# cczls1991/DL_Biomass

Hardware: NVIDIA B200
Metric: train tree-clouds/sec @10k pts (higher is better)
Workload: dtype bf16

## Files before the change

### dl_biomass_b200/csrc/sa_tc.cu

```cuda
#include <cuda.h>
#include <math.h>

#include "tc_common.cuh"

namespace b2pn {
namespace tc {

constexpr int R = 128;
constexpr int KC = 64;
constexpr int NUM_EPI = 256;
constexpr int NUM_LOAD = 128;
constexpr int LOAD_GROUPS = 2;
constexpr int MMA_WARP = (NUM_EPI + LOAD_GROUPS * NUM_LOAD) / 32;
constexpr int NT = NUM_EPI + LOAD_GROUPS * NUM_LOAD + 32;
constexpr int NT_TMA = 2 * NUM_EPI + 64;
constexpr int PROD_WARP_TMA = MMA_WARP + 1;
constexpr int NT_WIDE = 2 * NUM_EPI + 32 + NUM_LOAD;
constexpr int B_BYTES = R * LINE_BYTES;

constexpr unsigned GI_NONE = 0x00ffffffu;
__device__ __forceinline__ int gi_seg(unsigned b) { return (int)(b & 0xffffffu); }
__device__ __forceinline__ bool gi_none(unsigned b) { return (b & 0xffffffu) == 0xffffffu; }
__device__ __forceinline__ int gi_slot0(unsigned b) { return (int)((b >> 24) & 7u) << 3; }
__device__ __forceinline__ int gi_nv(unsigned b) { return (int)((b >> 27) & 15u); }
// ... 422 lines not shown
#pragma unroll
        for (int b = 0; b < 2; ++b) {
            const int64_t r8 = r0 + b * 64;
            qraw2[b] = __ldg(src.rm.rgrp + (r8 >> 3));
            qdead2 |= (r8 >= src.rm.rows ? 1u : 0u) << b;
        }
    }
    __device__ __forceinline__ void no_tile() { qraw2[0] = qraw2[1] = GI_NONE, qdead2 = 3u; }
    __device__ __forceinline__ void shift_tiles()
    {
#pragma unroll
        for (int b = 0; b < 2; ++b) qraw1[b] = qraw2[b];
        qdead1 = qdead2;
    }
    __device__ __forceinline__ void advance_tile()
    {
#pragma unroll
        for (int b = 0; b < 2; ++b) qinf[b] = (((qdead1 >> b) & 1u) || gi_none(qraw1[b])) ? GI_NONE : qraw1[b];
    }
    __device__ __forceinline__ void prefetch_next_rows(int lt, int kc0, int kstep, int num_kc) const
    {
        if ((lt & 7) != 0) return;
#pragma unroll
        for (int b = 0; b < 2; ++b) {
            const unsigned w = qraw1[b];
            if (((qdead1 >> b) & 1u) || gi_none(w) || gi_nv(w) == 0 || gi_slot0(w) != 0) continue;
            const int64_t base = (int64_t)gi_seg(w) * src.C + (lt & 15) * 4;
            for (int kc = kc0; kc < num_kc; kc += kstep) {
                if (kc * KC + (lt & 15) * 4 >= src.C) break;
                asm volatile("prefetch.global.L2 [%0];" ::"l"(src.arg + base + kc * KC));
                asm volatile("prefetch.global.L2 [%0];" ::"l"(src.dout + base + kc * KC));
            }
        }
    }
    __device__ __forceinline__ void load(int kc, int lt, Item &it) const
    {
        const int ch4 = kc * KC + (lt & 15) * 4;
        it.first = 0u;
#pragma unroll
        for (int b = 0; b < 2; ++b) {
            src.load_quad(qinf[b], ch4, it.q[b]);
            it.first |= (src.starts(qinf[b], ch4) ? 1u : 0u) << b;
        }
    }
    __device__ __forceinline__ void store(uint8_t *B, int kc, int lt, const Item &it) const
    {
        const int ch4 = kc * KC + (lt & 15) * 4;
#pragma unroll
        for (int b = 0; b < 2; ++b)
            src.store_quad(it.q[b], (it.first >> b) & 1u, ch4, lt >> 4, smem_u32(B) + b * (64 * LINE_BYTES), (lt & 15) * 4);
    }
    __device__ __forceinline__ void begin_tile(int64_t tile, int lt)
    {
        row0 = tile * R + (lt & 1) * 64;
        if (src.rm.seg_mode) {
#pragma unroll
            for (int g = 0; g < 8; ++g) inf[g] = src.rm.info(row0 + g * 8);
        } else {
#pragma unroll
            for (int g = 0; g < 8; ++g) inf[g] = src.rm.info_slots(row0 + g * 8);
        }
    }
    __device__ __forceinline__ void produce(uint8_t *B, int kc, int lt) const
    {
        const int cl = lt >> 1, nb = lt & 1;
        uint8_t *dst = B + nb * (64 * LINE_BYTES);
        const int ch = kc * KC + cl;
        uint4 v[8];
#pragma unroll
        for (int g = 0; g < 8; ++g) v[g] = src.chunk_i(ch, row0 + g * 8, inf[g]);
#pragma unroll
        for (int g = 0; g < 8; ++g) *reinterpret_cast<uint4 *>(dst + line_chunk_off(cl, g)) = v[g];
    }
    static __device__ __forceinline__ uint64_t b_desc(uint32_t b_saddr, int ks)
    {
        return smem_desc_sw128(b_saddr + ks * (16 * LINE_BYTES), 64 * LINE_BYTES, ATOM_BYTES);
    }
};

struct TmaFeatLoader {
    static constexpr bool B_MN = true;
    static constexpr bool USES_TMA = true;
    static constexpr bool WIDE = true;
    __device__ __forceinline__ void resolve(int64_t) {}
    __device__ __forceinline__ void begin_tile(int64_t, int) {}
    __device__ __forceinline__ void produce_tma(uint8_t *B, int64_t tile, int kc, const TmaMap *map, uint64_t *bar) const
    {
        mbar_expect_tx(bar, B_BYTES);
        tma_load_2d(B, map, (int)(tile * R), kc * KC, bar);
        tma_load_2d(B + 64 * LINE_BYTES, map, (int)(tile * R + 64), kc * KC, bar);
    }
    static __device__ __forceinline__ uint64_t b_desc(uint32_t b_saddr, int ks)
    {
        return smem_desc_sw128(b_saddr + ks * (16 * LINE_BYTES), 64 * LINE_BYTES, ATOM_BYTES);
    }
};

struct EpCtx {
    uint8_t *stage;
    const TmaMap *m0;
    const TmaMap *m1;
    uint64_t *bar;
    int64_t next_tile;
    int next_ch;
};
constexpr int EPI_STAGE_PER_WARP = 2 * 32 * LINE_BYTES;

__device__ __forceinline__ void stage_chunk(uint8_t *tile32, int lane, int g, const uint4 &v)
{
    *reinterpret_cast<uint4 *>(tile32 + lane * LINE_BYTES + ((g ^ (lane & 7)) << 4)) = v;
}
__device__ __forceinline__ uint4 unstage_chunk(const uint8_t *tile32, int lane, int g)
{
    return *reinterpret_cast<const uint4 *>(tile32 + lane * LINE_BYTES + ((g ^ (lane & 7)) << 4));
}

struct StoreF32Ep {
    static constexpr bool STAGED = false;
    float *out;
    int C;
    int64_t ld;
    __device__ __forceinline__ void resolve(int64_t) {}
    __device__ __forceinline__ void begin() {}
    __device__ __forceinline__ void tile_mt(uint32_t taddr, int64_t tile, int ch, int mt, int half, const EpCtx &cx)
    {
#pragma unroll 1
        for (int cc = half * 2; cc < half * 2 + 2; ++cc) {
            float v[32];
            tmem_ld32(taddr + cc * 32, v);
            if (ch < C) {
                float4 *dst = reinterpret_cast<float4 *>(out + (int64_t)ch * ld + tile * R + cc * 32);
#pragma unroll
                for (int j = 0; j < 8; ++j) dst[j] = make_float4(v[4 * j], v[4 * j + 1], v[4 * j + 2], v[4 * j + 3]);
            }
        }
    }
    __device__ __forceinline__ void finish_mt(int ch, int mt, int half) {}
};

template <int MT>
struct StatsEpTC {
    static constexpr bool STAGED = false;
    int C;
    double *partial;
    int cpad;
    int nslot;
    double S[MT], Q[MT];
    __device__ __forceinline__ void resolve(int64_t) {}
    __device__ __forceinline__ void begin()
    {
#pragma unroll
        for (int i = 0; i < MT; ++i) S[i] = Q[i] = 0.0;
    }
    __device__ __forceinline__ void tile_mt(uint32_t taddr, int64_t tile, int ch, int mt, int half, const EpCtx &cx)
    {
        float s = 0.f, q = 0.f;
#pragma unroll 1
        for (int cc = half * 2; cc < half * 2 + 2; ++cc) {
            float v[32];
            tmem_ld32(taddr + cc * 32, v);
#pragma unroll
            for (int j = 0; j < 32; ++j) {
                s += v[j];
                q = fmaf(v[j], v[j], q);
            }
        }
        S[mt] += (double)s;
        Q[mt] += (double)q;
    }
    __device__ __forceinline__ void finish_mt(int ch, int mt, int slot)
    {
        if (ch < C) {
            double *pt = partial + ((int64_t)blockIdx.x * nslot + slot) * 2 * cpad;
            pt[ch] = S[mt];
            pt[cpad + ch] = Q[mt];
        }
    }
};

// ... 269 lines not shown
        float *st = reinterpret_cast<float *>(cx.stage);
        __syncwarp();
#pragma unroll 1
        for (int cc = 0; cc < 2; ++cc) {
            float v[32];
            tmem_ld32(taddr + (half * 2 + cc) * 32, v);
#pragma unroll
            for (int j = 0; j < 32; ++j) {
                const int r = cc * 32 + j;
                st[r * 32 + ((((lane >> 2) ^ (r & 7))) << 2) + (lane & 3)] = v[j];
            }
        }
        __syncwarp();
        const bool vec = (C & 3) == 0;
#pragma unroll 1
        for (int rr = 0; rr < 2; ++rr) {
            const int r = rr * 32 + lane;
            const int64_t row = tile * R + half * 64 + r;
            if (row >= rm.rows) continue;
            int64_t dst = row;
            if (!rm.seg_mode) {
                const int sidx = __ldg(rm.row_src + row);
                if (sidx < 0) continue;
                dst = sidx;
            }
            float *base = dx + dst * C + ch0;
#pragma unroll
            for (int c4 = 0; c4 < 8; ++c4) {
                if (ch0 + c4 * 4 >= C) break;
                const float4 q = *reinterpret_cast<const float4 *>(st + r * 32 + ((c4 ^ (r & 7)) << 2));
                if (dxi != nullptr && !rm.seg_mode) {
                    const float e[4] = {q.x, q.y, q.z, q.w};
                    unsigned long long *acc = reinterpret_cast<unsigned long long *>(dxi + dst * C + ch0 + c4 * 4);
#pragma unroll
                    for (int k = 0; k < 4; ++k) {
                        if (ch0 + c4 * 4 + k >= C) break;
                        if (e[k] != 0.f) atomicAdd(acc + k, (unsigned long long)__float2ll_rn(e[k] * FIXED_ONE));
                    }
                } else if (vec) {
                    if (rm.seg_mode) {
                        *reinterpret_cast<float4 *>(base + c4 * 4) = q;
                    } else if (q.x != 0.f || q.y != 0.f || q.z != 0.f || q.w != 0.f) {
                        asm volatile("red.global.add.v4.f32 [%0], {%1, %2, %3, %4};" ::"l"(base + c4 * 4), "f"(q.x), "f"(q.y), "f"(q.z),
                                     "f"(q.w)
                                     : "memory");
                    }
                } else {
                    const float e[4] = {q.x, q.y, q.z, q.w};
#pragma unroll
                    for (int k = 0; k < 4; ++k) {
                        if (ch0 + c4 * 4 + k >= C) break;
                        if (rm.seg_mode) base[c4 * 4 + k] = e[k];
                        else if (e[k] != 0.f) atomicAdd(base + c4 * 4 + k, e[k]);
                    }
                }
            }
        }
    }
    __device__ __forceinline__ void finish_mt(int ch, int mt, int half) {}
};

template <int MT, bool STAGED, bool TMA>
struct SmemPlan {
    static constexpr int A_BYTES = MT * 128 * LINE_BYTES;
    static constexpr int STAGE_BYTES = A_BYTES + B_BYTES;
    static constexpr int EPI_WARPS = (TMA ? 2 : 1) * (NUM_EPI / 32);
    static constexpr int STAGES = !STAGED ? (MT == 1 ? 5 : 4) : (TMA ? (MT == 1 ? 3 : 2) : (MT == 1 ? 4 : 3));
    static constexpr int EPI_OFF = STAGES * STAGE_BYTES;
    static constexpr int EPI_BYTES = STAGED ? EPI_WARPS * EPI_STAGE_PER_WARP : 0;
    static constexpr int BAR_OFF = EPI_OFF + EPI_BYTES;
    static constexpr int TOTAL = BAR_OFF + 256 + 1024;
};

template <class BL, class = void>
struct LoaderPipelined { static constexpr bool value = false; };
template <class BL>
struct LoaderPipelined<BL, decltype((void)BL::PIPELINED)> { static constexpr bool value = BL::PIPELINED; };

template <class BL, class = void>
struct LoaderGroupsWide { static constexpr int value = 1; };
template <class BL>
struct LoaderGroupsWide<BL, decltype((void)BL::PIPE_GROUPS)> { static constexpr int value = BL::PIPELINED ? BL::PIPE_GROUPS : 1; };
template <class BL>
constexpr int gemm_threads() { return BL::USES_TMA ? NT_TMA : (BL::WIDE ? NT_WIDE + (LoaderGroupsWide<BL>::value - 1) * NUM_LOAD : NT); }

template <int MT, class BL, class EP>
__global__ void __launch_bounds__(gemm_threads<BL>(), 1)
    tc_rows_gemm_kernel(const GemmParams gp, BL bl, EP ep, const __grid_constant__ TmaMap tmap, const __grid_constant__ TmaMap tmap_e0,
                        const __grid_constant__ TmaMap tmap_e1)
{
    constexpr bool TMA = BL::USES_TMA;
    constexpr bool WIDE = BL::WIDE;
    static_assert(!TMA || WIDE, "TMA-fed kernels use the wide layout");
    constexpr int EPI_GROUPS = WIDE ? 2 : 1;
    constexpr int EPI_WARPS = EPI_GROUPS * (NUM_EPI / 32);
    constexpr int LGROUPS = WIDE ? LoaderGroupsWide<BL>::value : LOAD_GROUPS;
    constexpr int LOAD_T0 = WIDE ? (MMA_WARP + 1) * 32 : NUM_EPI;
    constexpr int NLOAD = NUM_LOAD;
    using P = SmemPlan<MT, EP::STAGED, WIDE>;
    extern __shared__ uint8_t smem_raw[];
    uint8_t *smem = reinterpret_cast<uint8_t *>((reinterpret_cast<uintptr_t>(smem_raw) + 1023) & ~(uintptr_t)1023);
    uint64_t *full = reinterpret_cast<uint64_t *>(smem + P::BAR_OFF);
    uint64_t *empty = full + P::STAGES;
    uint64_t *tfull = empty + P::STAGES;
    uint64_t *tempty = tfull + 2;
    uint64_t *ebar = tempty + 2;
    uint32_t *tmem_holder = reinterpret_cast<uint32_t *>(ebar + EPI_WARPS);

    const int tid = threadIdx.x, warp = tid >> 5, lane = tid & 31;
    const int mg = blockIdx.y;
    constexpr int TCOLS = MT * R * 2;
    const int64_t rows = gp.rows_dev ? *gp.rows_dev : gp.rows;
    const int64_t num_tiles = (rows + R - 1) / R;
    bl.resolve(rows);
    ep.resolve(rows);

    if (tid == 0) {
        for (int s = 0; s < P::STAGES; ++s) {
            mbar_init(&full[s], TMA ? 1 : NLOAD);
            mbar_init(&empty[s], 1);
        }
        for (int a = 0; a < 2; ++a) {
            mbar_init(&tfull[a], 1);
            mbar_init(&tempty[a], NUM_EPI);
        }
        for (int w = 0; w < EPI_WARPS; ++w) mbar_init(&ebar[w], 1);
        fence_barrier_init();
    }
    if (warp == MMA_WARP) tmem_alloc<TCOLS>(tmem_holder);
    tc_fence_before();
    __syncthreads();
    tc_fence_after();
    const uint32_t tmem_base = *tmem_holder;

    if (TMA && warp == PROD_WARP_TMA) {
        if constexpr (TMA) {
            if (lane == 0) {
                uint32_t it = 0;
                for (int64_t tile = blockIdx.x; tile < num_tiles; tile += gridDim.x) {
                    for (int kc = 0; kc < gp.num_kc; ++kc, ++it) {
                        const int s = it % P::STAGES;
                        const uint32_t ph = (it / P::STAGES) & 1u;
                        mbar_wait(&empty[s], ph ^ 1u);
                        uint8_t *A = smem + s * P::STAGE_BYTES;
                        uint8_t *B = A + P::A_BYTES;
                        mbar_expect_tx(&full[s], P::A_BYTES);
                        bulk_g2s(A, gp.a_packed + ((int64_t)mg * gp.num_kc + kc) * P::A_BYTES, P::A_BYTES, &full[s]);
                        bl.produce_tma(B, tile, kc, &tmap, &full[s]);
                        mbar_arrive(&full[s]);
                    }
                }
            }
        }
    } else if (!TMA && tid >= LOAD_T0 && tid < LOAD_T0 + LGROUPS * NLOAD) {
        if constexpr (!TMA) {
            const int g = (tid - LOAD_T0) / NLOAD;
            const int lt = (tid - LOAD_T0) % NLOAD;
            if constexpr (LoaderPipelined<BL>::value) {
                typename BL::Item cur, nxt;
                const int num_kc = gp.num_kc;
                const int64_t my_tiles = blockIdx.x < num_tiles ? (num_tiles - blockIdx.x + gridDim.x - 1) / gridDim.x : 0;
                const int64_t items = my_tiles * num_kc;
                const int tstep = num_kc >= LGROUPS ? 1 : LGROUPS / num_kc;
                auto tile_of = [&](int64_t tl) { return (int64_t)blockIdx.x + tl * gridDim.x; };
                auto fetch_or_none = [&](int64_t tl) {
                    if (tl < my_tiles) bl.fetch_tile(tile_of(tl), lt);
                    else bl.no_tile();
                };
                int64_t i = g;
                if (i < items) {
                    int64_t tl = i / num_kc;
                    int kc = (int)(i % num_kc);
                    bl.fetch_tile(tile_of(tl), lt);
                    bl.shift_tiles();
                    bl.advance_tile();
                    bl.load(kc, lt, cur);
                    fetch_or_none(tl + tstep);
                    bl.shift_tiles();
                    bl.prefetch_next_rows(lt, num_kc % LGROUPS == 0 ? g : 0, num_kc % LGROUPS == 0 ? LGROUPS : 1, num_kc);
                    fetch_or_none(tl + 2 * tstep);
                    auto item = [&](typename BL::Item &c, typename BL::Item &n) -> bool {
                        const int64_t ni = i + LGROUPS;
                        const bool has_next = ni < items;
                        int nkc = kc + LGROUPS;
                        int64_t ntl = tl;
                        while (nkc >= num_kc) {
                            nkc -= num_kc;
                            ++ntl;
                        }
                        if (has_next) {
                            if (ntl != tl) bl.advance_tile();
                            bl.load(nkc, lt, n);
                            if (ntl != tl) {
                                bl.shift_tiles();
                                bl.prefetch_next_rows(lt, num_kc % LGROUPS == 0 ? g : 0, num_kc % LGROUPS == 0 ? LGROUPS : 1, num_kc);
                                fetch_or_none(ntl + 2 * tstep);
                            }
                        }
                        const int s = (int)(i % P::STAGES);
                        const uint32_t ph = (uint32_t)(i / P::STAGES) & 1u;
                        mbar_wait(&empty[s], ph ^ 1u);
                        uint8_t *A = smem + s * P::STAGE_BYTES;
                        uint8_t *B = A + P::A_BYTES;
                        if (lt == 0) {
                            mbar_expect_tx(&full[s], P::A_BYTES);
                            bulk_g2s(A, gp.a_packed + ((int64_t)mg * num_kc + kc) * P::A_BYTES, P::A_BYTES, &full[s]);
                        }
                        RouteSource::zero_tile<NLOAD>(smem_u32(B), B_BYTES, lt);
                        RouteSource::group_barrier<NLOAD>(1 + g);
                        bl.store(B, kc, lt, c);
                        fence_proxy_async_smem();
                        mbar_arrive(&full[s]);
                        i = ni;
                        kc = nkc;
                        tl = ntl;
                        return has_next;
                    };
                    while (item(cur, nxt) && item(nxt, cur)) {
                    }
                }
            } else {
                uint32_t it = 0;
                int64_t cur_tile = -1;
                for (int64_t tile = blockIdx.x; tile < num_tiles; tile += gridDim.x) {
                    for (int kc = 0; kc < gp.num_kc; ++kc, ++it) {
                        if ((int)(it % LGROUPS) != g) continue;
                        if (tile != cur_tile) {
                            bl.begin_tile(tile, lt);
                            cur_tile = tile;
                        }
                        const int s = it % P::STAGES;
                        const uint32_t ph = (it / P::STAGES) & 1u;
                        mbar_wait(&empty[s], ph ^ 1u);
// ... 685 lines not shown
        bn[c] = (float)mean;
        bn[cmax + c] = (float)rstd;
        bn[2 * cmax + c] = (float)scale;
        bn[3 * cmax + c] = (float)((double)beta[c] - mean * scale);
    }
}

__global__ void bn_bwd_finalize_tc_kernel(const double *partial, int gx, int C, int cpad, const CountArg count, int training,
                                          float *grad_gamma, float *grad_beta, float *sbar)
{
    const int c = (blockIdx.x * blockDim.x + threadIdx.x) >> 5;
    if (c >= C) return;
    double S, Q;
    warp_sum_partials(partial, gx, cpad, c, S, Q);
    if ((threadIdx.x & 31) == 0) {
        const double E = count.get();
        if (grad_beta) grad_beta[c] = (float)S;
        if (grad_gamma) grad_gamma[c] = (float)Q;
        sbar[c] = (training && E > 0) ? (float)(S / E) : 0.f;
        sbar[C + c] = (training && E > 0) ? (float)(Q / E) : 0.f;
    }
}

template <bool CLOUDS>
__global__ void route_grad_tc_kernel(RowMapTC rm, const int64_t *rows_dev, const float *dout, const int32_t *arg, int C, int64_t ld,
                                     __nv_bfloat16 *dh)
{
    if (rows_dev) rm.rows = *rows_dev;
    const int64_t groups = (rm.rows + 127) / 128 * 16;
    const int64_t total = groups * C;
    for (int64_t i = (int64_t)blockIdx.x * blockDim.x + threadIdx.x; i < total; i += (int64_t)gridDim.x * blockDim.x) {
        const int ch = (int)(i / groups);
        const int64_t g = i - (int64_t)ch * groups;
        const unsigned inf = rm.info(g * 8);
        uint4 v = make_uint4(0u, 0u, 0u, 0u);
        if (CLOUDS) {
            float f[8];
            bool any = false;
#pragma unroll
            for (int e = 0; e < 8; ++e) {
                const int64_t row = g * 8 + e;
                f[e] = 0.f;
                if (e < gi_nv(inf)) {
                    const int64_t sg = __ldg(rm.batch + row);
                    if ((int64_t)__ldg(arg + sg * C + ch) == row) {
                        f[e] = __ldg(dout + sg * C + ch);
                        any = true;
                    }
                }
            }
            if (any) v = pack8(f);
        } else if (gi_nv(inf) > 0) {
            const int64_t m = gi_seg(inf);
            const int a = __ldg(arg + m * C + ch) - gi_slot0(inf);
            if (a >= 0 && a < 8) {
                const unsigned short gb = __bfloat16_as_ushort(__float2bfloat16(__ldg(dout + m * C + ch)));
                const unsigned w = (a & 1) ? ((unsigned)gb << 16) : (unsigned)gb;
                const int q = a >> 1;
                v.x = q == 0 ? w : 0u;
                v.y = q == 1 ? w : 0u;
                v.z = q == 2 ? w : 0u;
                v.w = q == 3 ? w : 0u;
            }
        }
        *reinterpret_cast<uint4 *>(dh + (int64_t)ch * ld + g * 8) = v;
    }
}

__global__ void bn_bwd_apply_tc_kernel(RowMapTC rm, const int64_t *rows_dev, __nv_bfloat16 *dz, const __nv_bfloat16 *z, int C,
                                       int64_t ld, const float *scale, const float *sbar)
{
    if (rows_dev) rm.rows = *rows_dev;
    const int64_t groups = (rm.rows + 127) / 128 * 16;
    const int64_t total = groups * C;
    for (int64_t i = (int64_t)blockIdx.x * blockDim.x + threadIdx.x; i < total; i += (int64_t)gridDim.x * blockDim.x) {
        const int ch = (int)(i / groups);
        const int64_t r8 = (i - (int64_t)ch * groups) * 8;
        const int nv = rm.valid8(r8);
        uint4 *p = reinterpret_cast<uint4 *>(dz + (int64_t)ch * ld + r8);
        if (nv == 0) {
            *p = make_uint4(0u, 0u, 0u, 0u);
            continue;
        }
        float d[8], zf[8];
        unpack8(*p, d);
        unpack8h(__ldg(reinterpret_cast<const uint4 *>(z + (int64_t)ch * ld + r8)), zf);
        const float sc = scale[ch];
        const float s1 = sbar[ch], s2 = sbar[C + ch];
#pragma unroll
        for (int e = 0; e < 8; ++e) d[e] = e < nv ? sc * (d[e] - s1 - zf[e] * s2) : 0.f;
        *p = pack8(d);
    }
}

struct DwReduceJob {
    const float *partial;
    int splits, n_out, k_total, use_map;
    InCols cols;
    int k_true, ones_idx;
    float *grad_w, *grad_b;
};
struct DwReduceJobs {
    DwReduceJob j[3];
};
__global__ void dw_reduce_flat_tc_kernel(const DwReduceJobs jobs)
{
    const DwReduceJob &jb = jobs.j[blockIdx.y];
    const int k_true = jb.k_true, k_total = jb.k_total, n_out = jb.n_out, splits = jb.splits;
    const int64_t i = (int64_t)blockIdx.x * blockDim.x + threadIdx.x;
    if (i >= (int64_t)n_out * (k_true + 1)) return;
    const int n = (int)(i / (k_true + 1));
    const int k = (int)(i - (int64_t)n * (k_true + 1));
    int c0 = -1, c1 = -1;
    if (k == k_true) {
        c0 = jb.ones_idx;
    } else if (!jb.use_map) {
        c0 = k;
    } else {
        const int nx = jb.cols.nx();
        if (k < jb.cols.c_in) {
            c0 = k;
            c1 = jb.cols.x_f32 ? k + jb.cols.c_in : -1;
        } else {
            c0 = nx + (k - jb.cols.c_in);
            c1 = c0 + 3;
        }
    }
    const int64_t stride = (int64_t)n_out * k_total;
    const float *base = jb.partial + (int64_t)n * k_total;
    constexpr int U = 16;
    double acc[U];
#pragma unroll
    for (int u = 0; u < U; ++u) acc[u] = 0.0;
    int p = 0;
    for (; p + U <= splits; p += U) {
#pragma unroll
        for (int u = 0; u < U; ++u) {
            const float *row = base + (int64_t)(p + u) * stride;
            float v = row[c0];
            if (c1 >= 0) v += row[c1];
            acc[u] += (double)v;
        }
    }
    for (; p < splits; ++p) {
        const float *row = base + (int64_t)p * stride;
        acc[0] += (double)row[c0];
        if (c1 >= 0) acc[0] += (double)row[c1];
    }
#pragma unroll
    for (int w = U / 2; w > 0; w >>= 1)
#pragma unroll
        for (int u = 0; u < w; ++u) acc[u] += acc[u + w];
    const double sum = acc[0];
    if (k == k_true) {
        if (jb.grad_b) jb.grad_b[n] = (float)sum;
    } else if (jb.grad_w) {
        jb.grad_w[(int64_t)n * k_true + k] = (float)sum;
    }
}

constexpr int DWR_WARPS = 8;
constexpr int DWR_MAX_SPLITS = 160;
__global__ void __launch_bounds__(32 * DWR_WARPS) dw_reduce_tc_kernel(const DwReduceJobs jobs)
{
    const DwReduceJob &jb = jobs.j[blockIdx.y];
    const int k_true = jb.k_true, k_total = jb.k_total, n_out = jb.n_out, splits = jb.splits;
    const int w = threadIdx.y;
    const int64_t i = (int64_t)blockIdx.x * 32 + threadIdx.x;
    const bool live = i < (int64_t)n_out * (k_true + 1);
    const int n = live ? (int)(i / (k_true + 1)) : 0;
    const int k = live ? (int)(i - (int64_t)n * (k_true + 1)) : 0;
    int c0 = 0, c1 = -1;
    if (k == k_true) {
        c0 = jb.ones_idx;
// ... 562 lines not shown
    for (int i = 0; i < 3; ++i) {
        dj.j[i] = jobs[i < n ? i : 0];
        const int64_t tot = (int64_t)dj.j[i].n_out * (dj.j[i].k_true + 1);
        mx = tot > mx ? tot : mx;
    }
    if (mx <= 16384)
        dw_reduce_tc_kernel<<<dim3((unsigned)((mx + 31) / 32), (unsigned)n), dim3(32, DWR_WARPS), 0, st>>>(dj);
    else
        dw_reduce_flat_tc_kernel<<<dim3((unsigned)((mx + 127) / 128), (unsigned)n), 128, 0, st>>>(dj);
    note_launch();
}

int sa_backward_bf16(const b2pn_sa_args &a, const b2pn_sa_grads &g, cudaStream_t st)
{
    int rc = check_args_tc(a);
    if (rc) return rc;
    if (!g.grad_out) return B2PN_EINVAL;
    const ShapesTC s = shapes_tc(a);
    if (a.n_dst == 0 || s.rows == 0) return B2PN_OK;
    if (a.workspace_bytes < sa_workspace_bytes_bf16(a, 1) || !a.workspace) return B2PN_EINVAL;
    WsTC ws(a.workspace);
    BwdWsTC b = carve_bwd_tc(a, s, ws);
    const RowMapTC rm = rowmap_tc(a, s);
    const RowsArg ra = rowsarg_tc(a, s);
    const __nv_bfloat16 *z1 = (const __nv_bfloat16 *)a.h1, *z2 = (const __nv_bfloat16 *)a.h2;
    float *bn1 = a.bn, *bn2 = a.bn + 4 * s.cmax;
    const bool need_dx = g.grad_x != nullptr && a.c_in > 0;

    {
        const PackJob jobs[3] = {pack_job(a.mlp.w[2], s.c2, s.c3, 1, s.c2, nullptr, b.pkT[2]),
                                 pack_job(a.mlp.w[1], s.c1, s.c2, 1, s.c1, nullptr, b.pkT[1]),
                                 pack_job(a.mlp.w[0], a.c_in, s.c1, 1, s.c0, nullptr, b.pkT[0])};
        launch_packs(jobs, need_dx ? 3 : 2, st);
    }
    const CountArg count = {a.seg_mode == B2PN_SEG_SLOTS ? a.num_rows + 1 : nullptr, (double)s.rows};

    MaskSumsStoreEpTC<1> e31 = {s.c2, a.mlp.gamma[1], a.mlp.beta[1], a.mlp.act, b.partial, s.cpad, 4};
    MaskSumsStoreEpTC<2> e32 = {s.c2, a.mlp.gamma[1], a.mlp.beta[1], a.mlp.act, b.partial, s.cpad, 4};
    TmaMap mdz2, mz2;
    if ((rc = make_tma_feature_major(&mdz2, b.dz2, s.c2, s.ld, 32))) return rc;
    if ((rc = make_tma_feature_major(&mz2, z2, s.c2, s.ld, 32))) return rc;
    LineFillK<FeatSource<1>> xa2 = {{rm, z2, s.c2, s.ld, a.mlp.act, s.c2, a.mlp.gamma[1], a.mlp.beta[1], FMT_BF16}};
    TmaMap map_v = kNoMap, map_a1 = kNoMap, map_a2 = kNoMap;
    const bool tma_x = a.row_valid != nullptr;
    const bool tma_x2 = tma_x && s.c2 % 64 == 0 && (s.c2 % 256) + 16 <= 256, tma_x1 = tma_x && s.c1 % 64 == 0 && (s.c1 % 256) + 16 <= 256;
    if (tma_x2 || tma_x1) {
        if ((rc = make_tma_row_valid(&map_v, a.row_valid, s.ld))) return rc;
    }
    const bool x_from_z = a.a1 == nullptr;
    if (x_from_z && !(tma_x1 && tma_x2 && a.seg_mode == B2PN_SEG_SLOTS)) return B2PN_EINVAL;
    if (tma_x2 && (rc = make_tma_feature_major(&map_a2, x_from_z ? (const void *)z2 : a.a2, s.c2, s.ld))) return rc;
    if (tma_x1 && (rc = make_tma_feature_major(&map_a1, x_from_z ? (const void *)z1 : a.a1, s.c1, s.ld))) return rc;
    if (a.seg_mode == B2PN_SEG_CLOUDS) {
        route_grad_tc_kernel<true><<<apply_grid(s.ld, s.c3), 256, 0, st>>>(rm, ra.dev, g.grad_out, a.arg, s.c3, s.ld, b.dh3);
        note_launch();
        TmaMap map3;
        if ((rc = make_tma_feature_major(&map3, b.dh3, s.c3, s.ld))) return rc;
        TmaFeatLoader bl;
        if ((rc = launch_by_mt(b.pkT[2], ra, bl, e31, e32, st, map3, mdz2, mz2))) return rc;
        TmaSource y3 = {rm};
        if (tma_x2) {
            TmaFill xt = {s.c2, 1, nullptr, nullptr, 0};
            rc = launch_dw(y3, xt, s.c3, s.c2 + 1, s, ra, b.dwp[2], st, map3, map_a2, map_v);
        } else {
            rc = launch_dw(y3, xa2, s.c3, s.c2 + 1, s, ra, b.dwp[2], st, map3);
        }
        if (rc) return rc;
    } else {
        const int vec = (s.c3 % 4 == 0 && ((uintptr_t)g.grad_out | (uintptr_t)a.arg) % 16 == 0) ? 1 : 0;
        RouteSource rs = {rm, g.grad_out, a.arg, s.c3, vec};
        FeatLoaderTC<RouteSource, true> bl = {rs};
        if ((rc = launch_by_mt(b.pkT[2], ra, bl, e31, e32, st, kNoMap, mdz2, mz2))) return rc;
        if (tma_x2) {
            TmaFill xt = {s.c2, 1, x_from_z ? a.mlp.gamma[1] : nullptr, a.mlp.beta[1], a.mlp.act};
            rc = launch_dw(rs, xt, s.c3, s.c2 + 1, s, ra, b.dwp[2], st, kNoMap, map_a2, map_v);
        } else {
            rc = launch_dw(rs, xa2, s.c3, s.c2 + 1, s, ra, b.dwp[2], st);
        }
        if (rc) return rc;
    }
    bn_bwd_finalize_tc_kernel<<<(s.c2 + 3) / 4, 128, 0, st>>>(b.partial, 4 * grid_x_for(b.pkT[2], s.tiles), s.c2, s.cpad, count,
                                                                 a.training, g.grad_gamma[1], g.grad_beta[1], b.sbar);
    note_launch();
    {
        bn_bwd_apply_tc_kernel<<<apply_grid(s.ld, s.c2), 256, 0, st>>>(rm, ra.dev, b.dz2, z2, s.c2, s.ld, bn2 + 2 * s.cmax, b.sbar);
        note_launch();
    }
    TmaMap map2, map1;
    if ((rc = make_tma_feature_major(&map2, b.dz2, s.c2, s.ld))) return rc;
    if ((rc = make_tma_feature_major(&map1, b.dz1, s.c1, s.ld))) return rc;
    TmaSource y2 = {rm};
    {
        TmaFeatLoader bl;
        MaskSumsStoreEpTC<1> e1 = {s.c1, a.mlp.gamma[0], a.mlp.beta[0], a.mlp.act, b.partial, s.cpad, 4};
        MaskSumsStoreEpTC<2> e2 = {s.c1, a.mlp.gamma[0], a.mlp.beta[0], a.mlp.act, b.partial, s.cpad, 4};
        TmaMap mdz1, mz1;
        if ((rc = make_tma_feature_major(&mdz1, b.dz1, s.c1, s.ld, 32))) return rc;
        if ((rc = make_tma_feature_major(&mz1, z1, s.c1, s.ld, 32))) return rc;
        if ((rc = launch_by_mt(b.pkT[1], ra, bl, e1, e2, st, map2, mdz1, mz1))) return rc;
        if (tma_x1) {
            TmaFill xt = {s.c1, 1, x_from_z ? a.mlp.gamma[0] : nullptr, a.mlp.beta[0], a.mlp.act};
            rc = launch_dw(y2, xt, s.c2, s.c1 + 1, s, ra, b.dwp[1], st, map2, map_a1, map_v);
        } else {
            LineFillK<FeatSource<1>> xa1 = {{rm, z1, s.c1, s.ld, a.mlp.act, s.c1, a.mlp.gamma[0], a.mlp.beta[0], FMT_BF16}};
            rc = launch_dw(y2, xa1, s.c2, s.c1 + 1, s, ra, b.dwp[1], st, map2);
        }
        if (rc) return rc;
    }
    bn_bwd_finalize_tc_kernel<<<(s.c1 + 3) / 4, 128, 0, st>>>(b.partial, 4 * grid_x_for(b.pkT[1], s.tiles), s.c1, s.cpad, count,
                                                                 a.training, g.grad_gamma[0], g.grad_beta[0], b.sbar);
    note_launch();
    {
        bn_bwd_apply_tc_kernel<<<apply_grid(s.ld, s.c1), 256, 0, st>>>(rm, ra.dev, b.dz1, z1, s.c1, s.ld, bn1 + 2 * s.cmax, b.sbar);
        note_launch();
    }
    TmaSource y1 = {rm};
    {
        if (l1_materialised(a, s)) {
            TmaMap map_g1;
            if ((rc = make_tma_feature_major(&map_g1, a.g1, s.k1 + 1, s.ld))) return rc;
            TmaFill xt = {s.k1 + 1, 0, nullptr, nullptr, 0};
            rc = launch_dw(y1, xt, s.c1, s.k1 + 1, s, ra, b.dwp[0], st, map1, map_g1, kNoMap);
        } else {
            LineFillGather xg = {{rm, a.x, s.cols, a.pos_src, a.pos_dst, s.k1, FMT_BF16}};
            rc = launch_dw(y1, xg, s.c1, s.k1 + 1, s, ra, b.dwp[0], st, map1);
        }
        if (rc) return rc;
        const DwReduceJob jobs[3] = {dw_reduce_job(b.dwp[2], s.c3, s.c2 + 1, nullptr, s.c2, s.c2, s, g.grad_w[2], g.grad_b[2]),
                                     dw_reduce_job(b.dwp[1], s.c2, s.c1 + 1, nullptr, s.c1, s.c1, s, g.grad_w[1], g.grad_b[1]),
                                     dw_reduce_job(b.dwp[0], s.c1, s.k1 + 1, &s.cols, s.c0, s.k1, s, g.grad_w[0], g.grad_b[0])};
        launch_dw_reduces(jobs, 3, st);
    }
    if (need_dx) {
        TmaFeatLoader bl;
        const int64_t nx = a.n_src * (int64_t)a.c_in;
        if (b.dxi) B2PN_CUDA(cudaMemsetAsync(b.dxi, 0, (size_t)nx * sizeof(long long), st));
        else if (a.seg_mode == B2PN_SEG_SLOTS) B2PN_CUDA(cudaMemsetAsync(g.grad_x, 0, (size_t)nx * sizeof(float), st));
        ScatterEpTC e = {rm, g.grad_x, a.c_in, b.dxi};
        if ((rc = launch_by_mt(b.pkT[0], ra, bl, e, e, st, map1))) return rc;
        if (b.dxi) {
            fixed_to_f32_kernel<<<(unsigned)((nx + 255) / 256), 256, 0, st>>>(b.dxi, g.grad_x, nx);
            note_launch();
        }
    }
    B2PN_LAUNCH_CHECK();
    return B2PN_OK;
}

}
}
```

Before: 5922.

## Fold BN backward apply into TMA-fed GEMM loader via converter warps

Adds a TmaApplyLoader whose extra 128 converter threads wait for the TMA-landed dz tile in shared memory, apply the batch-norm backward transform in place using z, and write the result back to global memory when mg==0. The next GEMM then consumes the converted tile, so the separate bn_bwd_apply kernel launches for layers 2 and 1 are skipped whenever the consuming GEMM has a single M-group. This removes a full read/write pass over dz and two kernel launches. In exchange the pipeline gains an extra barrier hop and conversion latency per stage, the dx GEMM is reordered ahead of the dW computation, and the block gets more threads.

New measurement: 5601 (median of 6 runs). 0.946x the previous value.

```diff
diff --git a/dl_biomass_b200/csrc/sa_tc.cu b/dl_biomass_b200/csrc/sa_tc.cu
--- a/dl_biomass_b200/csrc/sa_tc.cu
+++ b/dl_biomass_b200/csrc/sa_tc.cu
@@ -528,6 +528,7 @@
     static constexpr bool B_MN = true;
     static constexpr bool USES_TMA = true;
     static constexpr bool WIDE = true;
+    static constexpr bool CONVERT = false;
     __device__ __forceinline__ void resolve(int64_t) {}
     __device__ __forceinline__ void begin_tile(int64_t, int) {}
     __device__ __forceinline__ void produce_tma(uint8_t *B, int64_t tile, int kc, const TmaMap *map, uint64_t *bar) const
@@ -541,6 +542,63 @@
         return smem_desc_sw128(b_saddr + ks * (16 * LINE_BYTES), 64 * LINE_BYTES, ATOM_BYTES);
     }
 };
+
+__device__ __forceinline__ uint4 bn_bwd_dz8(const uint4 &graw, const uint4 &zraw, int nv, float sc, float s1, float s2)
+{
+    float d[8], zf[8];
+    unpack8(graw, d);
+    unpack8h(zraw, zf);
+#pragma unroll
+    for (int e = 0; e < 8; ++e) d[e] = e < nv ? sc * (d[e] - s1 - zf[e] * s2) : 0.f;
+    return pack8(d);
+}
+
+struct TmaApplyLoader : TmaFeatLoader {
+    static constexpr bool CONVERT = true;
+    RowMapTC rm;
+    __nv_bfloat16 *dz;
+    const __nv_bfloat16 *z;
+    int C;
+    int64_t ld;
+    const float *scale;
+    const float *sbar;
+    __device__ __forceinline__ void resolve(int64_t r) { rm.resolve(r); }
+    __device__ __forceinline__ void load_z(int64_t tile, int kc, int lt, uint4 (&zr)[8]) const
+    {
+        const int ch = kc * KC + (lt & 63);
+        const uint4 *p = reinterpret_cast<const uint4 *>(z + (int64_t)ch * ld + tile * R + (lt >> 6) * 64);
+#pragma unroll
+        for (int g = 0; g < 8; ++g) zr[g] = ch < C ? __ldg(p + g) : make_uint4(0u, 0u, 0u, 0u);
+    }
+    __device__ __forceinline__ void prefetch_z(int64_t tile, int kc, int lt) const
+    {
+        const int ch = kc * KC + (lt & 63);
+        if (ch < C) asm volatile("prefetch.global.L2 [%0];" ::"l"(z + (int64_t)ch * ld + tile * R + (lt >> 6) * 64));
+    }
+    __device__ __forceinline__ void convert(uint8_t *B, int64_t tile, int kc, int lt, const uint4 (&zr)[8], bool store) const
+    {
+        const int cl = lt & 63, ch = kc * KC + cl;
+        if (ch >= C) return;
+        const int64_t r0 = tile * R + (lt >> 6) * 64;
+        const unsigned nv64 = rm.valid64(r0);
+        const float sc = scale[ch], s1 = sbar[ch], s2 = sbar[C + ch];
+        uint8_t *line = B + (lt >> 6) * (64 * LINE_BYTES);
+        uint4 *gp = reinterpret_cast<uint4 *>(dz + (int64_t)ch * ld + r0);
+#pragma unroll
+        for (int g = 0; g < 8; ++g) {
+            uint4 *q = reinterpret_cast<uint4 *>(line + line_chunk_off(cl, g));
+            const int nv = (int)((nv64 >> (4 * g)) & 15u);
+            const uint4 v = nv == 0 ? make_uint4(0u, 0u, 0u, 0u) : bn_bwd_dz8(*q, zr[g], nv, sc, s1, s2);
+            *q = v;
+            if (store) gp[g] = v;
+        }
+    }
+};
+
+template <class BL, class = void>
+struct LoaderConverts { static constexpr bool value = false; };
+template <class BL>
+struct LoaderConverts<BL, decltype((void)BL::CONVERT)> { static constexpr bool value = BL::CONVERT; };
 
 struct EpCtx {
     uint8_t *stage;
@@ -976,7 +1034,11 @@
 template <class BL>
 struct LoaderGroupsWide<BL, decltype((void)BL::PIPE_GROUPS)> { static constexpr int value = BL::PIPELINED ? BL::PIPE_GROUPS : 1; };
 template <class BL>
-constexpr int gemm_threads() { return BL::USES_TMA ? NT_TMA : (BL::WIDE ? NT_WIDE + (LoaderGroupsWide<BL>::value - 1) * NUM_LOAD : NT); }
+constexpr int gemm_threads()
+{
+    return BL::USES_TMA ? NT_TMA + (LoaderConverts<BL>::value ? NUM_LOAD : 0)
+                        : (BL::WIDE ? NT_WIDE + (LoaderGroupsWide<BL>::value - 1) * NUM_LOAD : NT);
+}
 
 template <int MT, class BL, class EP>
 __global__ void __launch_bounds__(gemm_threads<BL>(), 1)
@@ -985,6 +1047,8 @@
 {
     constexpr bool TMA = BL::USES_TMA;
     constexpr bool WIDE = BL::WIDE;
+    constexpr bool CONV = LoaderConverts<BL>::value;
+    constexpr int CONV_T0 = NT_TMA;
     static_assert(!TMA || WIDE, "TMA-fed kernels use the wide layout");
     constexpr int EPI_GROUPS = WIDE ? 2 : 1;
     constexpr int EPI_WARPS = EPI_GROUPS * (NUM_EPI / 32);
@@ -999,7 +1063,9 @@
     uint64_t *tfull = empty + P::STAGES;
     uint64_t *tempty = tfull + 2;
     uint64_t *ebar = tempty + 2;
-    uint32_t *tmem_holder = reinterpret_cast<uint32_t *>(ebar + EPI_WARPS);
+    uint64_t *xland = ebar + EPI_WARPS;
+    uint32_t *tmem_holder = reinterpret_cast<uint32_t *>(xland + (CONV ? P::STAGES : 0));
+    static_assert(((CONV ? 3 : 2) * P::STAGES + 4 + EPI_WARPS) * 8 + 4 <= 256, "barrier area");
 
     const int tid = threadIdx.x, warp = tid >> 5, lane = tid & 31;
     const int mg = blockIdx.y;
@@ -1011,8 +1077,9 @@
 
     if (tid == 0) {
         for (int s = 0; s < P::STAGES; ++s) {
-            mbar_init(&full[s], TMA ? 1 : NLOAD);
+            mbar_init(&full[s], TMA ? 1 + (CONV ? NUM_LOAD : 0) : NLOAD);
             mbar_init(&empty[s], 1);
+            if (CONV) mbar_init(&xland[s], 1);
         }
         for (int a = 0; a < 2; ++a) {
             mbar_init(&tfull[a], 1);
@@ -1040,9 +1107,29 @@
                         uint8_t *B = A + P::A_BYTES;
                         mbar_expect_tx(&full[s], P::A_BYTES);
                         bulk_g2s(A, gp.a_packed + ((int64_t)mg * gp.num_kc + kc) * P::A_BYTES, P::A_BYTES, &full[s]);
-                        bl.produce_tma(B, tile, kc, &tmap, &full[s]);
+                        bl.produce_tma(B, tile, kc, &tmap, CONV ? &xland[s] : &full[s]);
                         mbar_arrive(&full[s]);
+                        if (CONV) mbar_arrive(&xland[s]);
                     }
+                }
+            }
+        }
+    } else if (CONV && tid >= CONV_T0) {
+        if constexpr (CONV) {
+            const int lt = tid - CONV_T0;
+            uint32_t it = 0;
+            for (int64_t tile = blockIdx.x; tile < num_tiles; tile += gridDim.x) {
+                for (int kc = 0; kc < gp.num_kc; ++kc, ++it) {
+                    const int s = it % P::STAGES;
+                    const uint32_t ph = (it / P::STAGES) & 1u;
+                    uint4 zr[8];
+                    bl.load_z(tile, kc, lt, zr);
+                    if (kc + 1 < gp.num_kc) bl.prefetch_z(tile, kc + 1, lt);
+                    else if (tile + gridDim.x < num_tiles) bl.prefetch_z(tile + gridDim.x, 0, lt);
+                    mbar_wait(&xland[s], ph);
+                    bl.convert(smem + s * P::STAGE_BYTES + P::A_BYTES, tile, kc, lt, zr, mg == 0);
+                    fence_proxy_async_smem();
+                    mbar_arrive(&full[s]);
                 }
             }
         }
@@ -1894,14 +1981,7 @@
             *p = make_uint4(0u, 0u, 0u, 0u);
             continue;
         }
-        float d[8], zf[8];
-        unpack8(*p, d);
-        unpack8h(__ldg(reinterpret_cast<const uint4 *>(z + (int64_t)ch * ld + r8)), zf);
-        const float sc = scale[ch];
-        const float s1 = sbar[ch], s2 = sbar[C + ch];
-#pragma unroll
-        for (int e = 0; e < 8; ++e) d[e] = e < nv ? sc * (d[e] - s1 - zf[e] * s2) : 0.f;
-        *p = pack8(d);
+        *p = bn_bwd_dz8(*p, __ldg(reinterpret_cast<const uint4 *>(z + (int64_t)ch * ld + r8)), nv, scale[ch], sbar[ch], sbar[C + ch]);
     }
 }
 
@@ -2630,7 +2710,9 @@
     bn_bwd_finalize_tc_kernel<<<(s.c2 + 3) / 4, 128, 0, st>>>(b.partial, 4 * grid_x_for(b.pkT[2], s.tiles), s.c2, s.cpad, count,
                                                                  a.training, g.grad_gamma[1], g.grad_beta[1], b.sbar);
     note_launch();
-    {
+    const bool fold2 = b.pkT[1].num_mg == 1;
+    const TmaApplyLoader al2 = {{}, rm, b.dz2, z2, s.c2, s.ld, bn2 + 2 * s.cmax, b.sbar};
+    if (!fold2) {
         bn_bwd_apply_tc_kernel<<<apply_grid(s.ld, s.c2), 256, 0, st>>>(rm, ra.dev, b.dz2, z2, s.c2, s.ld, bn2 + 2 * s.cmax, b.sbar);
         note_launch();
     }
@@ -2645,7 +2727,9 @@
         TmaMap mdz1, mz1;
         if ((rc = make_tma_feature_major(&mdz1, b.dz1, s.c1, s.ld, 32))) return rc;
         if ((rc = make_tma_feature_major(&mz1, z1, s.c1, s.ld, 32))) return rc;
-        if ((rc = launch_by_mt(b.pkT[1], ra, bl, e1, e2, st, map2, mdz1, mz1))) return rc;
+        if ((rc = fold2 ? launch_by_mt(b.pkT[1], ra, al2, e1, e2, st, map2, mdz1, mz1)
+                        : launch_by_mt(b.pkT[1], ra, bl, e1, e2, st, map2, mdz1, mz1)))
+            return rc;
         if (tma_x1) {
             TmaFill xt = {s.c1, 1, x_from_z ? a.mlp.gamma[0] : nullptr, a.mlp.beta[0], a.mlp.act};
             rc = launch_dw(y2, xt, s.c2, s.c1 + 1, s, ra, b.dwp[1], st, map2, map_a1, map_v);
@@ -2658,10 +2742,32 @@
     bn_bwd_finalize_tc_kernel<<<(s.c1 + 3) / 4, 128, 0, st>>>(b.partial, 4 * grid_x_for(b.pkT[1], s.tiles), s.c1, s.cpad, count,
                                                                  a.training, g.grad_gamma[0], g.grad_beta[0], b.sbar);
     note_launch();
-    {
+    const bool fold1 = need_dx && b.pkT[0].num_mg == 1;
+    if (!fold1) {
         bn_bwd_apply_tc_kernel<<<apply_grid(s.ld, s.c1), 256, 0, st>>>(rm, ra.dev, b.dz1, z1, s.c1, s.ld, bn1 + 2 * s.cmax, b.sbar);
         note_launch();
     }
+    auto launch_dx1 = [&]() -> int {
+        const int64_t nx = a.n_src * (int64_t)a.c_in;
+        if (b.dxi) B2PN_CUDA(cudaMemsetAsync(b.dxi, 0, (size_t)nx * sizeof(long long), st));
+        else if (a.seg_mode == B2PN_SEG_SLOTS) B2PN_CUDA(cudaMemsetAsync(g.grad_x, 0, (size_t)nx * sizeof(float), st));
+        ScatterEpTC e = {rm, g.grad_x, a.c_in, b.dxi};
+        int r;
+        if (fold1) {
+            const TmaApplyLoader al1 = {{}, rm, b.dz1, z1, s.c1, s.ld, bn1 + 2 * s.cmax, b.sbar};
+            r = launch_by_mt(b.pkT[0], ra, al1, e, e, st, map1);
+        } else {
+            TmaFeatLoader bl;
+            r = launch_by_mt(b.pkT[0], ra, bl, e, e, st, map1);
+        }
+        if (r) return r;
+        if (b.dxi) {
+            fixed_to_f32_kernel<<<(unsigned)((nx + 255) / 256), 256, 0, st>>>(b.dxi, g.grad_x, nx);
+            note_launch();
+        }
+        return 0;
+    };
+    if (fold1 && (rc = launch_dx1())) return rc;
     TmaSource y1 = {rm};
     {
         if (l1_materialised(a, s)) {
@@ -2679,18 +2785,7 @@
                                      dw_reduce_job(b.dwp[0], s.c1, s.k1 + 1, &s.cols, s.c0, s.k1, s, g.grad_w[0], g.grad_b[0])};
         launch_dw_reduces(jobs, 3, st);
     }
-    if (need_dx) {
-        TmaFeatLoader bl;
-        const int64_t nx = a.n_src * (int64_t)a.c_in;
-        if (b.dxi) B2PN_CUDA(cudaMemsetAsync(b.dxi, 0, (size_t)nx * sizeof(long long), st));
-        else if (a.seg_mode == B2PN_SEG_SLOTS) B2PN_CUDA(cudaMemsetAsync(g.grad_x, 0, (size_t)nx * sizeof(float), st));
-        ScatterEpTC e = {rm, g.grad_x, a.c_in, b.dxi};
-        if ((rc = launch_by_mt(b.pkT[0], ra, bl, e, e, st, map1))) return rc;
-        if (b.dxi) {
-            fixed_to_f32_kernel<<<(unsigned)((nx + 255) / 256), 256, 0, st>>>(b.dxi, g.grad_x, nx);
-            note_launch();
-        }
-    }
+    if (need_dx && !fold1 && (rc = launch_dx1())) return rc;
     B2PN_LAUNCH_CHECK();
     return B2PN_OK;
 }
```
